# matheusfalcaopinto/triple-hybrid-rag

Measured on AMD Instinct MI355X. Metric: queries/sec (fused top-10), higher is better.
Workload: dtype f16 MFMA shortlist scan (f32 accumulate) + f64 rescoring of the f32 rows

## Files before the change

### triple-hybrid-rag_amd/_native.py

```python
from __future__ import annotations

import ctypes as C
import os
from typing import Optional, Tuple

import torch

from . import _build

THR_FLAG_CERTIFIED = 1
THR_FLAG_OVERFLOW = 2
THR_FLAG_EXACT = 4
THR_DENSE_MAX_K = 256
THR_BM25_MAX_TERMS = 32
THR_BM25_MAX_QUERIES = 1 << 20
THR_GRAPH_MAX_SEEDS = 16
THR_RRF_MAX_PER_CHANNEL = 128
THR_TOPK_MAX = 128
ABI_VERSION = 9

_lib = None


class NativeError(RuntimeError):
# ... 148 lines not shown
def _alloc_out(nq: int, k: int, device):
    tile = torch.empty((2, nq, k), dtype=torch.int64, device=device)
    return (tile[0].view(torch.float64), tile[1],
            torch.empty(nq, dtype=torch.int32, device=device),
            torch.empty(nq, dtype=torch.int32, device=device))


def _coll(doc_coll, query_coll, n: int, nq: int):
    if query_coll is None:
        return None, None
    if doc_coll is None:
        raise NativeError("query_coll without doc_coll")
    if doc_coll.shape != (n,) or query_coll.shape != (nq,):
        raise NativeError("doc_coll / query_coll have the wrong length")
    return _dev(doc_coll, torch.int32, "doc_coll", 1), _dev(query_coll, torch.int32, "query_coll", 1)


def dense_topk(docs, dnorm, inv_norm, queries, k: int, kprime: int, id_base: int = 0,
               workspace: Optional[torch.Tensor] = None, doc_coll=None, query_coll=None):
    pd = _dev(docs, torch.float32, "docs", 2)
    n, d = docs.shape
    pq = _dev(queries, torch.float32, "queries", 2)
    nq = queries.shape[0]
    if queries.shape[1] != d:
        raise NativeError(f"queries dim {queries.shape[1]} != docs dim {d}")
    pn = _dev(dnorm, torch.float64, "dnorm", 1)
    pi = _dev(inv_norm, torch.float32, "inv_norm", 1)
    if dnorm.shape[0] != n or inv_norm.shape[0] != n:
        raise NativeError("dnorm / inv_norm length != n_docs")
    need = dense_workspace_bytes(n, d, nq, kprime)
    if workspace is None or workspace.numel() * workspace.element_size() < need:
        workspace = torch.empty(need, dtype=torch.uint8, device=docs.device)
    pw = _dev(workspace, workspace.dtype, "workspace")
    S, I, cnt, flg = _alloc_out(nq, k, docs.device)
    pdc, pqc = _coll(doc_coll, query_coll, n, nq)
    _check(load().thr_dense_topk(pd, pn, pi, n, d, id_base, pq, nq, k, kprime, pdc, pqc, S.data_ptr(),
                                 I.data_ptr(), cnt.data_ptr(), flg.data_ptr(), pw,
                                 workspace.numel() * workspace.element_size(), _stream()),
           "thr_dense_topk")
    return S, I, cnt, flg


def dense_topk_exact(docs, dnorm, queries, k: int, id_base: int = 0, doc_coll=None, query_coll=None):
    pd = _dev(docs, torch.float32, "docs", 2)
    n, d = docs.shape
    pq = _dev(queries, torch.float32, "queries", 2)
    nq = queries.shape[0]
    if queries.shape[1] != d:
        raise NativeError(f"queries dim {queries.shape[1]} != docs dim {d}")
    pn = _dev(dnorm, torch.float64, "dnorm", 1)
    if dnorm.shape[0] != n:
        raise NativeError("dnorm length != n_docs")
    need = int(load().thr_dense_exact_workspace_bytes(n, nq))
    ws = torch.empty(need, dtype=torch.uint8, device=docs.device)
    S, I, cnt, flg = _alloc_out(nq, k, docs.device)
    pdc, pqc = _coll(doc_coll, query_coll, n, nq)
    _check(load().thr_dense_topk_exact(pd, pn, n, d, id_base, pq, nq, k, pdc, pqc, S.data_ptr(),
                                       I.data_ptr(), cnt.data_ptr(), flg.data_ptr(),
                                       ws.data_ptr(), need, _stream()), "thr_dense_topk_exact")
    return S, I, cnt, flg


def dense_scan_probe(docs, inv_norm, queries, workspace: torch.Tensor) -> None:
    pd = _dev(docs, torch.float32, "docs", 2)
    n, d = docs.shape
    pq = _dev(queries, torch.float32, "queries", 2)
    if queries.shape[1] != d or inv_norm.shape[0] != n:
        raise NativeError("probe: shape mismatch")
    pi = _dev(inv_norm, torch.float32, "inv_norm", 1)
    pw = _dev(workspace, workspace.dtype, "workspace")
    _check(load().thr_dense_scan_probe(pd, pi, n, d, pq, queries.shape[0], pw,
                                       workspace.numel() * workspace.element_size(), _stream()),
           "thr_dense_scan_probe")


def dense_f16_query_tile(dim: int, packed: bool, n_queries: int) -> int:
    return int(load().thr_dense_f16_query_tile(dim, 1 if packed else 0, n_queries))


def dense_f16_max_queries(dim: int, packed: bool) -> int:
    return int(load().thr_dense_f16_max_queries(dim, 1 if packed else 0))


def dense_rescue_workspace_bytes(n_queries: int, k: int) -> int:
    return int(load().thr_dense_rescue_workspace_bytes(n_queries, k))


def dense_rescue(docs, dnorm, queries, S, I, cnt, flg, id_base: int = 0,
                 workspace: Optional[torch.Tensor] = None, doc_coll=None, query_coll=None) -> torch.Tensor:
    pd = _dev(docs, torch.float32, "docs", 2)
    pn = _dev(dnorm, torch.float64, "dnorm", 1)
    pq = _dev(queries, torch.float32, "queries", 2)
    n, d = docs.shape
    nq, k = I.shape
    need = int(load().thr_dense_rescue_workspace_bytes(nq, k))
    if workspace is None or workspace.numel() * workspace.element_size() < need:
        workspace = torch.empty(need, dtype=torch.uint8, device=docs.device)
    n_rescued = torch.zeros(1, dtype=torch.int32, device=docs.device)
    pdc, pqc = _coll(doc_coll, query_coll, n, nq)
    _check(load().thr_dense_rescue(pd, pn, n, d, id_base, pq, nq, k, pdc, pqc, S.data_ptr(), I.data_ptr(),
                                   cnt.data_ptr(), flg.data_ptr(), n_rescued.data_ptr(),
                                   workspace.data_ptr(),
                                   workspace.numel() * workspace.element_size(), _stream()),
           "thr_dense_rescue")
    return n_rescued


def dense_quantize_f16(docs: torch.Tensor, keep_copy: bool = True):
    p = _dev(docs, torch.float32, "docs", 2)
    n, d = docs.shape
    d16 = None
    if keep_copy:
        nbytes = int(load().thr_dense_f16_copy_bytes(n, d))
        d16 = torch.empty((nbytes // (2 * d), d), dtype=torch.float16, device=docs.device)
    err = torch.zeros(1, dtype=torch.float32, device=docs.device)
    _check(load().thr_dense_quantize_f16(p, n, d, d16.data_ptr() if keep_copy else None,
                                         err.data_ptr(), _stream()), "thr_dense_quantize_f16")
    return d16, float(err.item())


def dense_f16_layout(dim: int) -> str:
    return f"fragment-major/mfma{32 if os.environ.get('THR_DENSE_MFMA') == '32' else 16}/dim{dim}"


def dense_f16_workspace_bytes(n_docs: int, dim: int, n_queries: int, kprime: int) -> int:
    return int(load().thr_dense_f16_workspace_bytes(n_docs, dim, n_queries, kprime))


def dense_topk_f16(docs, docs16, doc_rel_err: float, dnorm, inv_norm, queries, k: int,
                   kprime: int, id_base: int = 0, workspace: Optional[torch.Tensor] = None,
                   doc_coll=None, query_coll=None):
    pd = _dev(docs, torch.float32, "docs", 2)
    ph = _dev(docs16, torch.float16, "docs16", 2) if docs16 is not None else None
    n, d = docs.shape
    if docs16 is not None and tuple(docs16.shape) != ((n + 31) // 32 * 32, d):
        raise NativeError("docs16 is not the fragment-major copy of docs (thr_dense_quantize_f16)")
    pq = _dev(queries, torch.float32, "queries", 2)
    nq = queries.shape[0]
    if queries.shape[1] != d:
        raise NativeError(f"queries dim {queries.shape[1]} != docs dim {d}")
    pn = _dev(dnorm, torch.float64, "dnorm", 1)
    pi = _dev(inv_norm, torch.float32, "inv_norm", 1)
    if dnorm.shape[0] != n or inv_norm.shape[0] != n:
        raise NativeError("dnorm / inv_norm length != n_docs")
    need = dense_f16_workspace_bytes(n, d, nq, kprime)
    if workspace is None or workspace.numel() * workspace.element_size() < need:
        workspace = torch.empty(need, dtype=torch.uint8, device=docs.device)
    pw = _dev(workspace, workspace.dtype, "workspace")
    S, I, cnt, flg = _alloc_out(nq, k, docs.device)
    pdc, pqc = _coll(doc_coll, query_coll, n, nq)
    _check(load().thr_dense_topk_f16(pd, ph, float(doc_rel_err), pn, pi, n, d, id_base, pq, nq, k,
                                     kprime, pdc, pqc, S.data_ptr(), I.data_ptr(), cnt.data_ptr(),
                                     flg.data_ptr(), pw,
                                     workspace.numel() * workspace.element_size(), _stream()),
           "thr_dense_topk_f16")
    return S, I, cnt, flg


def dense_shortlist_f16(docs, docs16, doc_rel_err: float, inv_norm, queries, kprime: int, m: int,
                        workspace: torch.Tensor, doc_coll=None, query_coll=None) -> torch.Tensor:
    pd = _dev(docs, torch.float32, "docs", 2)
    ph = _dev(docs16, torch.float16, "docs16", 2) if docs16 is not None else None
    n, d = docs.shape
    pq = _dev(queries, torch.float32, "queries", 2)
    nq = queries.shape[0]
    if queries.shape[1] != d or inv_norm.shape[0] != n:
        raise NativeError("shortlist: shape mismatch")
    pi = _dev(inv_norm, torch.float32, "inv_norm", 1)
    need = dense_f16_workspace_bytes(n, d, nq, kprime)
    if workspace.numel() * workspace.element_size() < need:
        raise NativeError("shortlist: workspace smaller than thr_dense_f16_workspace_bytes")
    pw = _dev(workspace, workspace.dtype, "workspace")
    pdc, pqc = _coll(doc_coll, query_coll, n, nq)
    lb = torch.empty((nq, m), dtype=torch.float32, device=docs.device)
    _check(load().thr_dense_shortlist_f16(pd, ph, float(doc_rel_err), pi, n, d, pq, nq, kprime, pdc, pqc,
                                          m, lb.data_ptr(), pw,
                                          workspace.numel() * workspace.element_size(), _stream()),
           "thr_dense_shortlist_f16")
    return lb


# ... 465 lines not shown
```

### triple-hybrid-rag_amd/csrc/dense.hip

```cpp
#include <stdlib.h>

#include "thr_common.hpp"

namespace thr {

constexpr int CHUNK = 256;
constexpr int MODE_ALL = 0, MODE_FILTER = 1;
constexpr int CAND_CAP = 16384;
constexpr int SAMPLE_MAX = 1 << 20;
constexpr int WBUF = 256;
constexpr int ROW_BITS = 27;
constexpr uint32_t ROW_MASK = (1u << ROW_BITS) - 1;
constexpr int ROW_BITS_F16 = 25;

struct Cand {
    float score;
    uint32_t doc;
};

}
struct ScanSlot {
    int qtile, slice, nslices;
};
__device__ __forceinline__ ScanSlot scan_slot(int n_qtiles) {
// ... 623 lines not shown
                [&](int u) { return fkey(load_cand(u).score); }, my_n, kprime, hist, bc);
            floor32 = fkey_inv(tkey);
            for (int u = 0; u < my_n; ++u) {
                const Cand e = load_cand(u);
                if (fkey(e.score) > tkey) {
                    const int p = atomicAdd(&n_sel, 1);
                    s_id[p] = e.doc;
                }
            }
            __syncthreads();
            for (int u = 0; u < my_n; ++u) {
                const Cand e = load_cand(u);
                if (fkey(e.score) == tkey) {
                    const int p = atomicAdd(&n_sel, 1);
                    if (p < kprime) s_id[p] = e.doc;
                }
            }
            __syncthreads();
            if (threadIdx.x == 0 && n_sel > kprime) n_sel = kprime;
        } else {
            for (int u = 0; u < my_n; ++u) {
                const Cand e = load_cand(u);
                if (e.score > -INFINITY) {
                    const int p = atomicAdd(&n_sel, 1);
                    s_id[p] = e.doc;
                }
            }
        }
    }
    __syncthreads();
    const int ns = n_sel;
    for (int i = threadIdx.x; i < ns; i += SEL_THREADS) sel_rows[(int64_t)q * CAPB + i] = s_id[i];
    if (threadIdx.x == 0) {
        sel_meta[4 * q + 0] = ns;
        sel_meta[4 * q + 1] = (int32_t)__float_as_uint(floor32);
        sel_meta[4 * q + 2] = overflow ? 1 : 0;
        sel_meta[4 * q + 3] = (int32_t)__float_as_uint(gF);
    }
}

constexpr int RR_WAVES = 2, RR_THREADS = 64 * RR_WAVES, RR_ROWS = 64;
static size_t rescore_lds_bytes(int dim) {
    return sizeof(double) * dim + sizeof(float4) * RR_WAVES * RR_ROWS * RS_STRIDE;
}
template <int U>
__device__ __forceinline__ double rescore_pass(const f32x4* (&rp)[8], f32x4* stage, const double* q64,
                                               int nchunk, int lane, int lrow, int lch) {
    constexpr int D = U >= 2 ? 16 / U : 8;
    f32x4 nxt[D][U];
#pragma unroll
    for (int dd = 0; dd < D; ++dd)
#pragma unroll
        for (int u = 0; u < U; ++u) nxt[dd][u] = rp[u][8 * dd];
    double dot = 0.0;
#pragma unroll 1
    for (int ck0 = 0; ck0 < nchunk; ck0 += D) {
#pragma unroll
        for (int dd = 0; dd < D; ++dd) {
            const int ck = ck0 + dd;
#pragma unroll
            for (int u = 0; u < U; ++u) stage[(lrow + 8 * u) * RS_STRIDE + lch] = nxt[dd][u];
            const int cn = ck + D < nchunk ? ck + D : nchunk - 1;
#pragma unroll
            for (int u = 0; u < U; ++u) nxt[dd][u] = rp[u][8 * cn];
            __builtin_amdgcn_fence(__ATOMIC_ACQ_REL, "wavefront");
            __builtin_amdgcn_wave_barrier();
            const f32x4* src = stage + lane * RS_STRIDE;
            const double* qv = q64 + 32 * ck;
#pragma unroll
            for (int ch = 0; ch < 8; ++ch) {
                const f32x4 x = src[ch];
                dot = __fma_rn((double)x.x, qv[4 * ch + 0], dot);
                dot = __fma_rn((double)x.y, qv[4 * ch + 1], dot);
                dot = __fma_rn((double)x.z, qv[4 * ch + 2], dot);
                dot = __fma_rn((double)x.w, qv[4 * ch + 3], dot);
            }
            __builtin_amdgcn_fence(__ATOMIC_ACQ_REL, "wavefront");
            __builtin_amdgcn_wave_barrier();
        }
    }
    return dot;
}

template <int NB>
__global__ __launch_bounds__(RR_THREADS, 3) void rescore_rank(
    const float* __restrict__ docs, const double* __restrict__ dnorm, int dim, int64_t id_base,
    const float* __restrict__ queries, int k, double eps32, double doc_relerr,
    const float* __restrict__ qerr, const int32_t* __restrict__ sel_rows,
    const int32_t* __restrict__ sel_meta, double* __restrict__ out_scores,
    int64_t* __restrict__ out_ids, int32_t* __restrict__ out_counts, uint32_t* __restrict__ out_flags) {
    const int q = blockIdx.x;
    const int ns = sel_meta[4 * q + 0];
    if (NB == THR_DENSE_MAX_K ? ns > THR_DENSE_MAX_K : ns <= THR_DENSE_MAX_K) return;
    const float floor32 = __uint_as_float((uint32_t)sel_meta[4 * q + 1]);
    const bool overflow = sel_meta[4 * q + 2] != 0;
    extern __shared__ float4 lds_sel[];
    __shared__ double s_s[NB], o_s[NB];
    __shared__ int64_t s_id[NB], o_id[NB];
    __shared__ double s_qn;
    __shared__ int n_valid;
    const int lane = threadIdx.x & 63, wave = threadIdx.x >> 6;
    const double eq = qerr ? (double)qerr[q] : 0.0;
    const double eps = eps32 + doc_relerr * (1.0 + eq) + eq;
    double* q64 = reinterpret_cast<double*>(lds_sel);
    for (int i = threadIdx.x; i < dim; i += RR_THREADS) q64[i] = (double)queries[(int64_t)q * dim + i];
    for (int i = threadIdx.x; i < NB; i += RR_THREADS) {
        s_s[i] = o_s[i] = -INFINITY;
        s_id[i] = i < ns ? (int64_t)sel_rows[(int64_t)q * SEL_BIG_BAND + i] : INT64_MAX;
        o_id[i] = INT64_MAX;
    }
    if (threadIdx.x == 0) n_valid = 0;
    __syncthreads();

    f32x4* stage = reinterpret_cast<f32x4*>(lds_sel + dim / 2) + wave * (RR_ROWS * RS_STRIDE);
    const f32x4* docs4 = reinterpret_cast<const f32x4*>(docs);
    const int lrow = lane >> 3, lch = lane & 7;
    const int cpr = dim / 4, nchunk = dim / 32;
    const f32x4* q4 = reinterpret_cast<const f32x4*>(queries + (int64_t)q * dim);
    const double dn_first = (int)threadIdx.x < ns ? dnorm[s_id[threadIdx.x]] : 0.0;
    for (int b0 = 0; b0 <= ns; b0 += RR_WAVES * RR_ROWS) {
        const int rem = ns - b0 - wave;
        if (rem < 0) continue;
        const f32x4* rp[8];
#pragma unroll
        for (int u = 0; u < 8; ++u) {
            int j = b0 + wave + RR_WAVES * (lrow + 8 * u);
            j = j < ns ? j : ns;
            rp[u] = (j < ns ? docs4 + s_id[j] * cpr : q4) + lch;
        }
        const int jm = b0 + wave + RR_WAVES * lane;
        const int groups = rem / RR_WAVES / 8 + 1;
        double dot;
        if (groups <= 1) dot = rescore_pass<1>(rp, stage, q64, nchunk, lane, lrow, lch);
        else if (groups <= 2) dot = rescore_pass<2>(rp, stage, q64, nchunk, lane, lrow, lch);
        else if (groups <= 4) dot = rescore_pass<4>(rp, stage, q64, nchunk, lane, lrow, lch);
        else dot = rescore_pass<8>(rp, stage, q64, nchunk, lane, lrow, lch);
        if (jm < ns) s_s[jm] = dot;
        else if (jm == ns) s_qn = __dsqrt_rn(dot);
    }
    __syncthreads();
    for (int p = threadIdx.x; p < ns; p += RR_THREADS) {
        const int64_t row = s_id[p];
        const double qn = s_qn, dn = p == (int)threadIdx.x ? dn_first : dnorm[row], dot = s_s[p];
        double sim = -INFINITY;
        if (dn > 0.0) sim = qn > 0.0 ? __ddiv_rn(dot, __dmul_rn(qn, dn)) : 0.0;
        s_s[p] = sim;
        s_id[p] = sim == -INFINITY ? INT64_MAX : row + id_base;
    }
    __syncthreads();
    for (int p = threadIdx.x; p < ns; p += RR_THREADS) {
        const double ms = s_s[p];
        const int64_t mi = s_id[p];
        if (mi == INT64_MAX) continue;
        int rank = 0;
        for (int i = 0; i < ns; ++i) rank += better(s_s[i], s_id[i], ms, mi) ? 1 : 0;
        o_s[rank] = ms;
        o_id[rank] = mi;
    }
    __syncthreads();

    int mine_valid = 0;
    for (int i = threadIdx.x; i < k; i += RR_THREADS) {
        const bool ok = o_s[i] > -INFINITY;
        mine_valid += ok ? 1 : 0;
        out_scores[(int64_t)q * k + i] = ok ? o_s[i] : -INFINITY;
        out_ids[(int64_t)q * k + i] = ok ? o_id[i] : -1;
    }
    if (mine_valid) atomicAdd(&n_valid, mine_valid);
    __syncthreads();
    if (threadIdx.x == 0) {
        const int valid = n_valid;
        uint32_t flag = overflow ? THR_FLAG_OVERFLOW : 0u;
        bool cert;
        if (overflow) {
            cert = false;
        } else if (floor32 == -INFINITY) {
            cert = true;
        } else {
            const float gF = __uint_as_float((uint32_t)sel_meta[4 * q + 3]);
            const bool own = valid >= k && s_qn > 0.0 && (o_s[k - 1] - (double)floor32 / s_qn) > eps;
            const bool all = gF > -INFINITY && s_qn > 0.0 &&
                             ((double)gF / s_qn - (double)floor32 / s_qn) > eps;
            cert = own || all;
        }
        out_flags[q] = flag | (cert ? THR_FLAG_CERTIFIED : 0u);
        out_counts[q] = valid;
    }
}

constexpr int EX_THREADS = 256;
constexpr int EX_CAP = 1024;
constexpr int EX_SLABS = 64;

__global__ __launch_bounds__(EX_THREADS) void exact_slab_topk(
    const float* __restrict__ docs, const double* __restrict__ dnorm, int64_t n_docs, int dim,
    const float* __restrict__ queries, int n_queries, int k, double* __restrict__ slab_s,
    int64_t* __restrict__ slab_id, const uint32_t* __restrict__ skip_certified,
    const int32_t* __restrict__ doc_coll, const int32_t* __restrict__ query_coll) {
    extern __shared__ float lds_qv[];
    __shared__ double b_s[EX_CAP];
    __shared__ int64_t b_id[EX_CAP];
    __shared__ int b_cnt;
    __shared__ double t_s;
    __shared__ int64_t t_id;
    __shared__ double s_qn;
    __shared__ unsigned long long s_todo;
    const int slab = blockIdx.x;
    {
        const int q = blockIdx.y + (int)threadIdx.x * (int)gridDim.y;
        const bool todo = threadIdx.x < 64 && q < n_queries &&
                          !(skip_certified && (skip_certified[q] & THR_FLAG_CERTIFIED));
        const unsigned long long m = __ballot(todo);
        if (threadIdx.x == 0) s_todo = m;
        __syncthreads();
    }
    for (unsigned long long todo = s_todo; todo; todo &= todo - 1) {
        const int q = blockIdx.y + (__ffsll((long long)todo) - 1) * (int)gridDim.y;
        __syncthreads();
        for (int i = threadIdx.x; i < dim; i += EX_THREADS) lds_qv[i] = queries[(int64_t)q * dim + i];
        __syncthreads();
        if (threadIdx.x == 0) s_qn = __dsqrt_rn(seq_dot_f64(lds_qv, lds_qv, dim));
        BlockTopK<EX_CAP, EX_THREADS> tk;
        tk.init(b_s, b_id, &b_cnt, &t_s, &t_id, k);
        const double qn = s_qn;
        const int qc = query_coll ? query_coll[q] : -1;
        const int64_t per = (n_docs + EX_SLABS - 1) / EX_SLABS;
        const int64_t lo = slab * per, hi = (lo + per < n_docs) ? lo + per : n_docs;
        for (int64_t base = lo; base < hi; base += EX_THREADS) {
            int64_t row = base + threadIdx.x;
            bool ok = row < hi;
            double sim = -INFINITY;
            if (ok) {
                double dn = dnorm[row];
                if (qc != -1 && doc_coll[row] != qc) dn = 0.0;
                if (dn > 0.0) {
                    double dot = seq_dot_f64(docs + row * dim, lds_qv, dim);
                    sim = qn > 0.0 ? __ddiv_rn(dot, __dmul_rn(qn, dn)) : 0.0;
                }
            }
            tk.push(ok && sim > -INFINITY, sim, row);
        }
        int n = tk.finish();
        for (int i = threadIdx.x; i < k; i += EX_THREADS) {
            int64_t o = ((int64_t)q * EX_SLABS + slab) * k + i;
            slab_s[o] = i < n ? b_s[i] : -INFINITY;
            slab_id[o] = i < n ? b_id[i] : INT64_MAX;
        }
    }
}
// ... 457 lines not shown
                          int n_queries, int k, int kprime, double* out_scores, int64_t* out_ids,
                          int32_t* out_counts, uint32_t* out_flags, char* ws, hipStream_t st,
                          const int32_t* doc_coll, const int32_t* query_coll, int phase = PIPE_ALL,
                          const float* gfloor = nullptr, float* top_lb = nullptr, int top_m = 0,
                          const float* lb_all = nullptr, int n_shards = 0) {
    float* tau = (float*)(ws + p.off_tau);
    const bool h = p.kind == KIND_F16;
    float* qerr = h ? (float*)(ws + p.off_qerr) : nullptr;
    int* cnt = (int*)(ws + p.off_cnt);
    int* tcnt = (int*)(ws + p.off_tcnt);
    Cand* cand = (Cand*)(ws + p.off_cand);
    Cand* tlist = (Cand*)(ws + p.off_tlist);
    float* sample = (float*)(ws + p.off_sample);
    _Float16* qfrag = (_Float16*)(ws + p.off_qfrag);
    int nseg = 0;
    auto scan = [&](bool all, int64_t units, int64_t stride, float* smp, int64_t ld) -> int {
        if (p.qreg)
            return all ? launch_scan_f16q<MODE_ALL>(dim, docs16, qfrag, p.ntiles, units, stride,
                                                    nullptr, nullptr, nullptr, smp, ld, st, nullptr,
                                                    nullptr, nullptr, n_queries)
                       : launch_scan_f16q<MODE_FILTER>(dim, docs16, qfrag, p.ntiles, units, stride,
                                                       tau, cnt, cand, nullptr, 0, st, &nseg, doc_coll,
                                                       query_coll, n_queries);
        if (h)
            return all ? launch_scan_f16<MODE_ALL>(dim, p.nq, docs, inv_norm, n_docs, queries,
                                                   n_queries, p.ntiles, units, stride, nullptr,
                                                   nullptr, nullptr, 0, smp, ld, st)
                       : launch_scan_f16<MODE_FILTER>(dim, p.nq, docs, inv_norm, n_docs, queries,
                                                      n_queries, p.ntiles, units, stride, tau, tcnt,
                                                      tlist, p.tile_cap, nullptr, 0, st, doc_coll, query_coll);
        return all ? launch_scan_mfma<MODE_ALL>(dim, docs, inv_norm, n_docs, queries, n_queries,
                                               p.ntiles, units, stride, nullptr, nullptr, nullptr,
                                               0, smp, ld, st)
                   : launch_scan_mfma<MODE_FILTER>(dim, docs, inv_norm, n_docs, queries, n_queries,
                                                  p.ntiles, units, stride, tau, tcnt, tlist,
                                                  p.tile_cap, nullptr, 0, st, doc_coll, query_coll);
    };
    int rc;
    const double u = 5.9604644775390625e-08;
    const double eps32 = h ? ((double)dim + 16.0) * u : scan_eps(dim);
    int32_t* sel_rows = (int32_t*)(ws + p.off_selrows);
    int32_t* sel_meta = (int32_t*)(ws + p.off_selmeta);
    if (phase == PIPE_FINISH) {
        if (p.qreg && (rc = launch_scan_f16q<MODE_FILTER, true>(dim, docs16, qfrag, p.ntiles, p.groups, 1,
                                                                 nullptr, nullptr, nullptr, nullptr, 0, st,
                                                                 &nseg)))
            return rc;
    } else {
    hipError_t e = hipMemsetAsync(cnt, 0, p.off_cand - p.off_cnt, st);
    if (e != hipSuccess) return (int)e;
    if (p.qreg && (rc = launch_pack_queries(dim, queries, n_queries, p.qpad, qfrag, qerr, st))) return rc;
    float* qerr_k2 = p.qreg ? nullptr : qerr;
    if (p.sampled) {
        if ((rc = scan(true, p.sample_groups, p.sample_stride, sample, p.sample_docs))) return rc;
        hipLaunchKernelGGL(kth_select, dim3(p.qpad), dim3(256), 0, st, sample, p.sample_docs,
                           (int)p.sample_docs, p.ksample, queries, n_queries, dim, tau, qerr_k2,
                           doc_coll, query_coll, p.unit, p.sample_stride, n_docs);
    } else {
        hipLaunchKernelGGL(kth_select, dim3(p.qpad), dim3(256), 0, st, (const float*)nullptr,
                           (int64_t)0, 0, p.ksample, queries, n_queries, dim, tau, qerr_k2,
                           doc_coll, query_coll, p.unit, (int64_t)1, n_docs);
    }
    if ((rc = launch_status())) return rc;
    if ((rc = scan(false, p.groups, 1, nullptr, 0))) return rc;
    if (!p.qreg) {
        hipLaunchKernelGGL(bucket_candidates, dim3(BUCKET_BLOCKS, p.ntiles), dim3(256), 0, st, tcnt,
                           tlist, p.tile_cap, p.qtile, p.row_bits, cnt, cand);
        if ((rc = launch_status())) return rc;
    }
    }
    if (phase == PIPE_SHORTLIST) {
        hipLaunchKernelGGL(select_band<true>, dim3(n_queries), dim3(SEL_THREADS), band_lds_bytes(dim), st,
                           dim, queries, tau, cnt, cand, tcnt, p.tile_cap, p.qtile, k, kprime, eps32,
                           doc_relerr, qerr, nseg, nseg ? CAND_CAP / nseg : 0, doc_coll, query_coll,
                           sel_rows, sel_meta, (const float*)nullptr, (const float*)nullptr, 0, 0, top_lb,
                           top_m);
        return launch_status();
    }
    hipLaunchKernelGGL(select_band<false>, dim3(n_queries), dim3(SEL_THREADS), band_lds_bytes(dim), st,
                       dim, queries, tau, cnt, cand, tcnt, p.tile_cap, p.qtile, k, kprime, eps32,
                       doc_relerr, qerr, nseg, nseg ? CAND_CAP / nseg : 0, doc_coll, query_coll,
                       sel_rows, sel_meta, gfloor, lb_all, n_shards, top_m, (float*)nullptr, 0);
    if ((rc = launch_status())) return rc;
    hipLaunchKernelGGL(rescore_rank<THR_DENSE_MAX_K>, dim3(n_queries), dim3(RR_THREADS),
                       rescore_lds_bytes(dim), st, docs, dnorm, dim, id_base, queries, k, eps32,
                       doc_relerr, qerr, sel_rows, sel_meta, out_scores, out_ids, out_counts, out_flags);
    if ((rc = launch_status())) return rc;
    hipLaunchKernelGGL(rescore_rank<SEL_BIG_BAND>, dim3(n_queries), dim3(RR_THREADS),
                       rescore_lds_bytes(dim), st, docs, dnorm, dim, id_base, queries, k, eps32,
                       doc_relerr, qerr, sel_rows, sel_meta, out_scores, out_ids, out_counts, out_flags);
    return launch_status();
}

static int dense_args_ok(const void* docs, const void* dnorm, const void* inv_norm,
                         const void* queries, const void* a, const void* b, const void* c,
                         const void* d, const void* ws, int64_t n_docs, int n_queries, int k,
                         int kprime) {
    THR_RETURN_IF(!docs || !dnorm || !inv_norm || !queries || !a || !b || !c || !d || !ws,
                  THR_ERR_INVALID);
    THR_RETURN_IF(n_docs <= 0 || n_queries <= 0 || k <= 0 || kprime < k ||
                      kprime > THR_DENSE_MAX_K,
                  THR_ERR_INVALID);
    return THR_OK;
}

extern "C" int thr_dense_topk(const float* docs, const double* dnorm, const float* inv_norm,
                              int64_t n_docs, int dim, int64_t id_base, const float* queries,
                              int n_queries, int k, int kprime, const int32_t* doc_coll,
                              const int32_t* query_coll, double* out_scores,
                              int64_t* out_ids, int32_t* out_counts, uint32_t* out_flags,
                              void* workspace, size_t workspace_bytes, thr_stream_t stream) {
    clear_status();
    int rc = dense_args_ok(docs, dnorm, inv_norm, queries, out_scores, out_ids, out_counts,
                           out_flags, workspace, n_docs, n_queries, k, kprime);
    if (rc) return rc;
    THR_RETURN_IF((query_coll != nullptr) != (doc_coll != nullptr), THR_ERR_INVALID);
    THR_RETURN_IF(dim <= 0 || dim % CHUNK != 0 || dim / CHUNK > 4, THR_ERR_UNSUPPORTED);
    THR_RETURN_IF(n_docs >= (int64_t)1 << ROW_BITS, THR_ERR_UNSUPPORTED);
    const DensePlan p = make_plan(n_docs, n_queries, kprime);
    THR_RETURN_IF(workspace_bytes < p.total, THR_ERR_WORKSPACE);
    return dense_pipeline(p, docs, nullptr, 0.0, dnorm, inv_norm, n_docs, dim, id_base, queries,
                          n_queries, k, kprime, out_scores, out_ids, out_counts, out_flags,
                          (char*)workspace, (hipStream_t)stream, doc_coll, query_coll);
}

extern "C" size_t thr_dense_f16_workspace_bytes(int64_t n_docs, int dim, int n_queries,
                                                int kprime) {
    if (n_docs <= 0 || n_queries <= 0) return 0;
    const size_t a = make_plan(n_docs, n_queries, kprime, KIND_F16, dim, false).total;
    const size_t b = make_plan(n_docs, n_queries, kprime, KIND_F16, dim, true).total;
    return a > b ? a : b;
}

extern "C" int thr_dense_f16_max_queries(int dim, int packed) {
    if (dim != 512 && dim != 768 && dim != 1024) return 0;
    return packed ? qreg_max_queries(dim) : INT32_MAX;
}

extern "C" int thr_dense_f16_query_tile(int dim, int packed, int n_queries) {
    if (dim != 512 && dim != 768 && dim != 1024) return 0;
    (void)n_queries;
    return packed ? qreg_qw(dim) * qreg_waves(dim) : 32 * f16_pick_nq(dim);
}

extern "C" size_t thr_dense_f16_copy_bytes(int64_t n_docs, int dim) {
    if (n_docs <= 0 || dim <= 0) return 0;
    return sizeof(_Float16) * (size_t)((n_docs + 31) / 32 * 32) * (size_t)dim;
}

extern "C" int thr_dense_quantize_f16(const float* docs, int64_t n_docs, int dim, uint16_t* docs16,
                                      float* max_rel_err, thr_stream_t stream) {
    clear_status();
    THR_RETURN_IF(!docs || !max_rel_err || n_docs <= 0 || dim <= 0, THR_ERR_INVALID);
    THR_RETURN_IF(dim % 64 != 0, THR_ERR_UNSUPPORTED);
    hipStream_t st = (hipStream_t)stream;
    hipError_t e = hipMemsetAsync(max_rel_err, 0, sizeof(float), st);
    if (e != hipSuccess) return (int)e;
    if (docs16) {
        THR_RETURN_IF(dim % 16 != 0, THR_ERR_UNSUPPORTED);
        const int64_t n_pad = (n_docs + 31) / 32 * 32;
        hipLaunchKernelGGL(quantize_f16_norm, dim3((unsigned)((n_pad + 3) / 4)), dim3(256), 0, st,
                           docs, n_docs, dim, qreg_shape(dim), reinterpret_cast<_Float16*>(docs16),
                           reinterpret_cast<unsigned int*>(max_rel_err));
        return launch_status();
    }
    hipLaunchKernelGGL(measure_f16_error, dim3((unsigned)((n_docs + 3) / 4)), dim3(256), 0, st, docs,
                       n_docs, dim, reinterpret_cast<unsigned int*>(max_rel_err));
    return launch_status();
}

extern "C" int thr_dense_topk_f16(const float* docs, const uint16_t* docs16, double doc_rel_err,
// ... 254 lines not shown
```

### triple-hybrid-rag_amd/csrc/rrf.hip

```cpp
#include "thr_common.hpp"

namespace thr {

constexpr int RRF_THREADS = 128;
constexpr int RRF_MAXC = THR_RRF_MAX_PER_CHANNEL;
constexpr int RRF_SLOTS = 512;

__device__ __forceinline__ int last_rank(const int64_t* l, int n, int64_t id) {
    int r = 0;
    for (int j = 0; j < n; ++j)
        if (l[j] == id) r = j + 1;
    return r;
}
__device__ __forceinline__ bool seen_before(const int64_t* l, int i, int64_t id) {
    for (int j = 0; j < i; ++j)
        if (l[j] == id) return true;
    return false;
}

constexpr int RRF_RAG2 = 0, RRF_STANDALONE = 1, RRF_TWO = 2;
__device__ __forceinline__ int occurrences(const int64_t* l, int n, int64_t id) {
    int c = 0;
    for (int j = 0; j < n; ++j) c += l[j] == id ? 1 : 0;
    return c;
}

template <int MODE>
__global__ __launch_bounds__(RRF_THREADS) void rrf_fuse_kernel(
    const int64_t* __restrict__ lex, int n_lex, const int64_t* __restrict__ sem, int n_sem,
    const int64_t* __restrict__ gra, int n_gra, double w_lex, double w_sem, double w_gra, int rrf_k,
    int top_k, int64_t* __restrict__ out_ids, double* __restrict__ out_scores,
    int32_t* __restrict__ out_ranks, int32_t* __restrict__ out_counts) {
    static_assert(RRF_THREADS == RRF_MAXC && RRF_THREADS == 2 * WAVE, "one thread per position");
    __shared__ int64_t L[3][RRF_MAXC];
    __shared__ int len[3];
    __shared__ int wave_new[3][2];
    __shared__ double s_s[RRF_SLOTS];
    __shared__ int64_t c_id[RRF_SLOTS];
    __shared__ int c_rank[RRF_SLOTS][3];
    __shared__ int order[RRF_SLOTS];

    const int q = blockIdx.x, t = threadIdx.x, lane = t & 63, wave = t >> 6;
    const int64_t* src[3] = {lex, sem, gra};
    const int width[3] = {lex ? n_lex : 0, sem ? n_sem : 0, gra ? n_gra : 0};
    if (t < 3) len[t] = width[t];
    __syncthreads();
    for (int ch = 0; ch < 3; ++ch) {
        const int64_t id = t < width[ch] ? src[ch][(int64_t)q * width[ch] + t] : -1;
        L[ch][t] = id;
        if (t < width[ch] && id < 0) atomicMin(&len[ch], t);
    }
    __syncthreads();

    bool nw[3];
    int within[3];
    for (int ch = 0; ch < 3; ++ch) {
        nw[ch] = false;
        if (t < len[ch]) {
            const int64_t id = L[ch][t];
            nw[ch] = !seen_before(L[ch], t, id);
            for (int e = 0; e < ch && nw[ch]; ++e)
                if (last_rank(L[e], len[e], id)) nw[ch] = false;
        }
        const uint64_t m = __ballot(nw[ch]);
        within[ch] = __popcll(m & ((1ull << lane) - 1ull));
        if (lane == 0) wave_new[ch][wave] = __popcll(m);
    }
    __syncthreads();
    int base = 0, n = 0;
    for (int ch = 0; ch < 3; ++ch) {
        const int here = base + (wave ? wave_new[ch][0] : 0) + within[ch];
        base += wave_new[ch][0] + wave_new[ch][1];
        if (!nw[ch]) continue;
        const int64_t id = L[ch][t];
        const int lr = last_rank(L[0], len[0], id);
        const int sr = last_rank(L[1], len[1], id);
        const int gr = last_rank(L[2], len[2], id);
        double score = 0.0;
        if (MODE == RRF_RAG2) {
            if (lr) score = __dadd_rn(score, __ddiv_rn(w_lex, (double)(rrf_k + lr)));
            if (sr) score = __dadd_rn(score, __ddiv_rn(w_sem, (double)(rrf_k + sr)));
            if (gr) score = __dadd_rn(score, __ddiv_rn(w_gra, (double)(rrf_k + gr)));
        } else {
            const double w[3] = {w_lex, w_sem, w_gra};
            const int rk[3] = {lr, sr, gr};
#pragma unroll
            for (int c = 0; c < 3; ++c)
                if (rk[c]) {
                    const double v = __dmul_rn(w[c], __ddiv_rn(1.0, (double)(rrf_k + rk[c])));
                    const int reps = (MODE == RRF_TWO && c == 0) ? 1 : occurrences(L[c], len[c], id);
                    for (int r = 0; r < reps; ++r) score = __dadd_rn(score, v);
                }
        }
        c_id[here] = id;
        c_rank[here][0] = lr;
        c_rank[here][1] = sr;
        c_rank[here][2] = gr;
        s_s[here] = score;
    }
    n = base;
    __syncthreads();
    for (int p = t; p < n; p += RRF_THREADS) {
        const double ms = s_s[p];
        int rank = 0;
        for (int j = 0; j < n; ++j) {
            const double o = s_s[j];
            rank += (o > ms || (o == ms && j < p)) ? 1 : 0;
        }
        order[rank] = p;
    }
    __syncthreads();
    for (int i = t; i < top_k; i += RRF_THREADS) {
        const bool ok = i < n;
        const int p = ok ? order[i] : 0;
        out_ids[(int64_t)q * top_k + i] = ok ? c_id[p] : -1;
        out_scores[(int64_t)q * top_k + i] = ok ? s_s[p] : -INFINITY;
        if (out_ranks)
            for (int c = 0; c < 3; ++c)
                out_ranks[((int64_t)q * top_k + i) * 3 + c] = ok ? c_rank[p][c] : 0;
    }
    if (t == 0) out_counts[q] = n < top_k ? n : top_k;
}

__global__ __launch_bounds__(RRF_THREADS) void rerank_order_kernel(
    const float* __restrict__ scores, int n_lists, int64_t list_stride,
    const int64_t* __restrict__ ids, const int32_t* __restrict__ counts, int n, int top_k,
    int64_t* __restrict__ out_ids, double* __restrict__ out_scores, int32_t* __restrict__ out_counts) {
    __shared__ double s_s[RRF_SLOTS];
    __shared__ int order[RRF_SLOTS];
    const int q = blockIdx.x, t = threadIdx.x;
    int cnt = counts ? counts[q] : n;
    cnt = cnt < n ? cnt : n;
    for (int p = t; p < cnt; p += RRF_THREADS) {
        float best = -INFINITY;
        for (int l = 0; l < n_lists; ++l) best = fmaxf(best, scores[(int64_t)l * list_stride + (int64_t)q * n + p]);
        s_s[p] = best > -INFINITY ? (double)best : 0.0;
    }
    __syncthreads();
    for (int p = t; p < cnt; p += RRF_THREADS) {
        const double ms = s_s[p];
        int rank = 0;
        for (int j = 0; j < cnt; ++j) {
            const double o = s_s[j];
            rank += (o > ms || (o == ms && j < p)) ? 1 : 0;
        }
        order[rank] = p;
    }
    __syncthreads();
    for (int i = t; i < top_k; i += RRF_THREADS) {
        const bool ok = i < cnt;
        const int p = ok ? order[i] : 0;
        out_ids[(int64_t)q * top_k + i] = ok ? ids[(int64_t)q * n + p] : -1;
        out_scores[(int64_t)q * top_k + i] = ok ? s_s[p] : -INFINITY;
    }
    if (t == 0) out_counts[q] = cnt < top_k ? cnt : top_k;
}

__global__ __launch_bounds__(RRF_THREADS) void fuse_post_kernel(
    const int64_t* __restrict__ ids, const double* __restrict__ scores,
    const int32_t* __restrict__ ranks, const int32_t* __restrict__ counts, int n,
    const double* __restrict__ lex_s, int n_lex, const double* __restrict__ sem_s, int n_sem,
    const double* __restrict__ gra_s, int n_gra, double safety_threshold, int denoise,
    double quantile, int normalize, int top_k, int64_t* __restrict__ out_ids,
    double* __restrict__ out_scores, int32_t* __restrict__ out_counts) {
    __shared__ double s_s[2][RRF_SLOTS];
    __shared__ int64_t s_id[2][RRF_SLOTS];
    __shared__ int wave_cnt[2];
    __shared__ double red[2][2];
    const int q = blockIdx.x, t = threadIdx.x, lane = t & 63, wave = t >> 6;
    int cnt = counts ? counts[q] : n;
    cnt = cnt < n ? cnt : n;
    auto compact = [&](int from, int m, auto keep) -> int {
        int base = 0;
        for (int b0 = 0; b0 < m; b0 += RRF_THREADS) {
            const int i = b0 + t;
            const bool k = i < m && keep(i);
            const uint64_t bal = __ballot(k);
            if (lane == 0) wave_cnt[wave] = __popcll(bal);
            __syncthreads();
            const int at = base + (wave ? wave_cnt[0] : 0) + __popcll(bal & ((1ull << lane) - 1ull));
            if (k) {
                s_s[from ^ 1][at] = s_s[from][i];
                s_id[from ^ 1][at] = s_id[from][i];
            }
            base += wave_cnt[0] + wave_cnt[1];
            __syncthreads();
        }
        return base;
    };
    const double* chs[3] = {lex_s, sem_s, gra_s};
    const int chw[3] = {n_lex, n_sem, n_gra};
    for (int i = t; i < cnt; i += RRF_THREADS) {
        s_s[0][i] = scores[(int64_t)q * n + i];
        s_id[0][i] = ids[(int64_t)q * n + i];
    }
    __syncthreads();
    int m = cnt, cur = 0;
    if (safety_threshold > 0.0 && ranks) {
        m = compact(0, cnt, [&](int i) {
            double best = 0.0;
            for (int c = 0; c < 3; ++c) {
                const int r = ranks[((int64_t)q * n + i) * 3 + c];
                if (r > 0 && chs[c]) {
                    const double v = chs[c][(int64_t)q * chw[c] + r - 1];
                    best = v > best ? v : best;
                }
            }
            return best >= safety_threshold;
        });
        cur = 1;
    }
    if (denoise && m >= 3) {
        const double v = __dmul_rn((double)(m - 1), quantile);
        int prev = (int)floor(v);
        prev = prev < 0 ? 0 : prev > m - 1 ? m - 1 : prev;
        const int next = prev + 1 > m - 1 ? m - 1 : prev + 1;
        const double g = __dsub_rn(v, (double)prev);
        const double a = s_s[cur][m - 1 - prev], bb = s_s[cur][m - 1 - next];
        const double diff = __dsub_rn(bb, a);
        const double cut = g >= 0.5 ? __dsub_rn(bb, __dmul_rn(diff, __dsub_rn(1.0, g)))
                                    : __dadd_rn(a, __dmul_rn(diff, g));
        __syncthreads();
        const int from = cur;
        m = compact(from, m, [&](int i) { return s_s[from][i] >= cut; });
        cur ^= 1;
    }
    if (top_k > 0 && m > top_k) m = top_k;
    double lo = 0.0, hi = 0.0;
    if (normalize && m > 0) {
        double mn = INFINITY, mx = -INFINITY;
// ... 115 lines not shown
```

Baseline: 737,100.

## Hash-dedupe RRF candidates, merge rescore kernels, pool zero counters

RRF fusion replaces quadratic linear scans for duplicate detection, last rank and occurrence counting with a shared-memory open-addressing hash table. The rank sort is register-blocked over several positions per thread. The two templated rescore_rank launches collapse into one kernel that uses 32-bit row ids and reuses the stage LDS for its outputs. A pooled zero tensor replaces a per-call torch.zeros allocation. Together these cut launches, allocation and O(n^2) work, at the cost of atomics in the hash insert and a pooled counter slice whose reuse must stay correct.

```diff
diff --git a/triple-hybrid-rag_amd/_native.py b/triple-hybrid-rag_amd/_native.py
--- a/triple-hybrid-rag_amd/_native.py
+++ b/triple-hybrid-rag_amd/_native.py
@@ -254,6 +254,17 @@
     return int(load().thr_dense_f16_max_queries(dim, 1 if packed else 0))
 
 
+_ZERO_POOL: dict = {}
+
+
+def _zero_i32(device) -> torch.Tensor:
+    pool = _ZERO_POOL.get(str(device))
+    if pool is None or pool[1] >= pool[0].numel():
+        pool = _ZERO_POOL[str(device)] = [torch.zeros(4096, dtype=torch.int32, device=device), 0]
+    pool[1] += 1
+    return pool[0][pool[1] - 1:pool[1]]
+
+
 def dense_rescue_workspace_bytes(n_queries: int, k: int) -> int:
     return int(load().thr_dense_rescue_workspace_bytes(n_queries, k))
 
@@ -268,7 +279,7 @@
     need = int(load().thr_dense_rescue_workspace_bytes(nq, k))
     if workspace is None or workspace.numel() * workspace.element_size() < need:
         workspace = torch.empty(need, dtype=torch.uint8, device=docs.device)
-    n_rescued = torch.zeros(1, dtype=torch.int32, device=docs.device)
+    n_rescued = _zero_i32(docs.device)
     pdc, pqc = _coll(doc_coll, query_coll, n, nq)
     _check(load().thr_dense_rescue(pd, pn, n, d, id_base, pq, nq, k, pdc, pqc, S.data_ptr(), I.data_ptr(),
                                    cnt.data_ptr(), flg.data_ptr(), n_rescued.data_ptr(),
diff --git a/triple-hybrid-rag_amd/csrc/dense.hip b/triple-hybrid-rag_amd/csrc/dense.hip
--- a/triple-hybrid-rag_amd/csrc/dense.hip
+++ b/triple-hybrid-rag_amd/csrc/dense.hip
@@ -729,7 +729,6 @@
     return dot;
 }
 
-template <int NB>
 __global__ __launch_bounds__(RR_THREADS, 3) void rescore_rank(
     const float* __restrict__ docs, const double* __restrict__ dnorm, int dim, int64_t id_base,
     const float* __restrict__ queries, int k, double eps32, double doc_relerr,
@@ -737,13 +736,15 @@
     const int32_t* __restrict__ sel_meta, double* __restrict__ out_scores,
     int64_t* __restrict__ out_ids, int32_t* __restrict__ out_counts, uint32_t* __restrict__ out_flags) {
     const int q = blockIdx.x;
-    const int ns = sel_meta[4 * q + 0];
-    if (NB == THR_DENSE_MAX_K ? ns > THR_DENSE_MAX_K : ns <= THR_DENSE_MAX_K) return;
+    constexpr int NB = SEL_BIG_BAND, NOUT = THR_DENSE_MAX_K;
+    const int ns = sel_meta[4 * q + 0] < NB ? sel_meta[4 * q + 0] : NB;
     const float floor32 = __uint_as_float((uint32_t)sel_meta[4 * q + 1]);
     const bool overflow = sel_meta[4 * q + 2] != 0;
     extern __shared__ float4 lds_sel[];
-    __shared__ double s_s[NB], o_s[NB];
-    __shared__ int64_t s_id[NB], o_id[NB];
+    __shared__ double s_s[NB];
+    __shared__ int32_t s_id[NB];
+    static_assert(sizeof(float4) * RR_WAVES * RR_ROWS * RS_STRIDE >= NOUT * (sizeof(double) + sizeof(int32_t)),
+                  "the ranked output fits the stage tiles");
     __shared__ double s_qn;
     __shared__ int n_valid;
     const int lane = threadIdx.x & 63, wave = threadIdx.x >> 6;
@@ -751,10 +752,9 @@
     const double eps = eps32 + doc_relerr * (1.0 + eq) + eq;
     double* q64 = reinterpret_cast<double*>(lds_sel);
     for (int i = threadIdx.x; i < dim; i += RR_THREADS) q64[i] = (double)queries[(int64_t)q * dim + i];
-    for (int i = threadIdx.x; i < NB; i += RR_THREADS) {
-        s_s[i] = o_s[i] = -INFINITY;
-        s_id[i] = i < ns ? (int64_t)sel_rows[(int64_t)q * SEL_BIG_BAND + i] : INT64_MAX;
-        o_id[i] = INT64_MAX;
+    for (int i = threadIdx.x; i < ns; i += RR_THREADS) {
+        s_s[i] = -INFINITY;
+        s_id[i] = sel_rows[(int64_t)q * SEL_BIG_BAND + i];
     }
     if (threadIdx.x == 0) n_valid = 0;
     __syncthreads();
@@ -773,7 +773,7 @@
         for (int u = 0; u < 8; ++u) {
             int j = b0 + wave + RR_WAVES * (lrow + 8 * u);
             j = j < ns ? j : ns;
-            rp[u] = (j < ns ? docs4 + s_id[j] * cpr : q4) + lch;
+            rp[u] = (j < ns ? docs4 + (int64_t)s_id[j] * cpr : q4) + lch;
         }
         const int jm = b0 + wave + RR_WAVES * lane;
         const int groups = rem / RR_WAVES / 8 + 1;
@@ -786,23 +786,31 @@
         else if (jm == ns) s_qn = __dsqrt_rn(dot);
     }
     __syncthreads();
+    double* o_s = reinterpret_cast<double*>(lds_sel + dim / 2);
+    int32_t* o_id = reinterpret_cast<int32_t*>(o_s + NOUT);
+    for (int i = threadIdx.x; i < NOUT; i += RR_THREADS) {
+        o_s[i] = -INFINITY;
+        o_id[i] = INT32_MAX;
+    }
     for (int p = threadIdx.x; p < ns; p += RR_THREADS) {
-        const int64_t row = s_id[p];
+        const int32_t row = s_id[p];
         const double qn = s_qn, dn = p == (int)threadIdx.x ? dn_first : dnorm[row], dot = s_s[p];
         double sim = -INFINITY;
         if (dn > 0.0) sim = qn > 0.0 ? __ddiv_rn(dot, __dmul_rn(qn, dn)) : 0.0;
         s_s[p] = sim;
-        s_id[p] = sim == -INFINITY ? INT64_MAX : row + id_base;
+        s_id[p] = sim == -INFINITY ? INT32_MAX : row;
     }
     __syncthreads();
     for (int p = threadIdx.x; p < ns; p += RR_THREADS) {
         const double ms = s_s[p];
-        const int64_t mi = s_id[p];
-        if (mi == INT64_MAX) continue;
+        const int32_t mi = s_id[p];
+        if (mi == INT32_MAX) continue;
         int rank = 0;
         for (int i = 0; i < ns; ++i) rank += better(s_s[i], s_id[i], ms, mi) ? 1 : 0;
-        o_s[rank] = ms;
-        o_id[rank] = mi;
+        if (rank < NOUT) {
+            o_s[rank] = ms;
+            o_id[rank] = mi;
+        }
     }
     __syncthreads();
 
@@ -811,7 +819,7 @@
         const bool ok = o_s[i] > -INFINITY;
         mine_valid += ok ? 1 : 0;
         out_scores[(int64_t)q * k + i] = ok ? o_s[i] : -INFINITY;
-        out_ids[(int64_t)q * k + i] = ok ? o_id[i] : -1;
+        out_ids[(int64_t)q * k + i] = ok ? (int64_t)o_id[i] + id_base : -1;
     }
     if (mine_valid) atomicAdd(&n_valid, mine_valid);
     __syncthreads();
@@ -1435,11 +1443,7 @@
                        doc_relerr, qerr, nseg, nseg ? CAND_CAP / nseg : 0, doc_coll, query_coll,
                        sel_rows, sel_meta, gfloor, lb_all, n_shards, top_m, (float*)nullptr, 0);
     if ((rc = launch_status())) return rc;
-    hipLaunchKernelGGL(rescore_rank<THR_DENSE_MAX_K>, dim3(n_queries), dim3(RR_THREADS),
-                       rescore_lds_bytes(dim), st, docs, dnorm, dim, id_base, queries, k, eps32,
-                       doc_relerr, qerr, sel_rows, sel_meta, out_scores, out_ids, out_counts, out_flags);
-    if ((rc = launch_status())) return rc;
-    hipLaunchKernelGGL(rescore_rank<SEL_BIG_BAND>, dim3(n_queries), dim3(RR_THREADS),
+    hipLaunchKernelGGL(rescore_rank, dim3(n_queries), dim3(RR_THREADS),
                        rescore_lds_bytes(dim), st, docs, dnorm, dim, id_base, queries, k, eps32,
                        doc_relerr, qerr, sel_rows, sel_meta, out_scores, out_ids, out_counts, out_flags);
     return launch_status();
diff --git a/triple-hybrid-rag_amd/csrc/rrf.hip b/triple-hybrid-rag_amd/csrc/rrf.hip
--- a/triple-hybrid-rag_amd/csrc/rrf.hip
+++ b/triple-hybrid-rag_amd/csrc/rrf.hip
@@ -6,24 +6,44 @@
 constexpr int RRF_MAXC = THR_RRF_MAX_PER_CHANNEL;
 constexpr int RRF_SLOTS = 512;
 
-__device__ __forceinline__ int last_rank(const int64_t* l, int n, int64_t id) {
-    int r = 0;
-    for (int j = 0; j < n; ++j)
-        if (l[j] == id) r = j + 1;
-    return r;
-}
-__device__ __forceinline__ bool seen_before(const int64_t* l, int i, int64_t id) {
-    for (int j = 0; j < i; ++j)
-        if (l[j] == id) return true;
-    return false;
+constexpr uint64_t RRF_EMPTY = ~0ull;
+
+__device__ __forceinline__ int rrf_slot(uint64_t* hkey, int64_t id) {
+    uint32_t h = ((uint32_t)id ^ (uint32_t)((uint64_t)id >> 32)) * 2654435761u >> (32 - __builtin_ctz(RRF_SLOTS));
+    for (;;) {
+        const uint64_t old = atomicCAS((unsigned long long*)&hkey[h], (unsigned long long)RRF_EMPTY,
+                                       (unsigned long long)id);
+        if (old == RRF_EMPTY || old == (uint64_t)id) return (int)h;
+        h = (h + 1) & (RRF_SLOTS - 1);
+    }
+}
+
+template <int NI>
+__device__ __forceinline__ void rrf_rank_sort(const double* s_s, int n, int* order, int t) {
+    double ms[NI];
+    int rank[NI];
+#pragma unroll
+    for (int i = 0; i < NI; ++i) {
+        const int p = t + i * RRF_THREADS;
+        ms[i] = p < n ? s_s[p] : 0.0;
+        rank[i] = 0;
+    }
+    for (int j = 0; j < n; j += 2) {
+        const double o0 = s_s[j], o1 = s_s[j + 1];
+        const bool two = j + 1 < n;
+#pragma unroll
+        for (int i = 0; i < NI; ++i) {
+            const int p = t + i * RRF_THREADS;
+            rank[i] += (o0 > ms[i] || (o0 == ms[i] && j < p)) ? 1 : 0;
+            rank[i] += (two && (o1 > ms[i] || (o1 == ms[i] && j + 1 < p))) ? 1 : 0;
+        }
+    }
+#pragma unroll
+    for (int i = 0; i < NI; ++i)
+        if (t + i * RRF_THREADS < n) order[rank[i]] = t + i * RRF_THREADS;
 }
 
 constexpr int RRF_RAG2 = 0, RRF_STANDALONE = 1, RRF_TWO = 2;
-__device__ __forceinline__ int occurrences(const int64_t* l, int n, int64_t id) {
-    int c = 0;
-    for (int j = 0; j < n; ++j) c += l[j] == id ? 1 : 0;
-    return c;
-}
 
 template <int MODE>
 __global__ __launch_bounds__(RRF_THREADS) void rrf_fuse_kernel(
@@ -32,36 +52,50 @@
     int top_k, int64_t* __restrict__ out_ids, double* __restrict__ out_scores,
     int32_t* __restrict__ out_ranks, int32_t* __restrict__ out_counts) {
     static_assert(RRF_THREADS == RRF_MAXC && RRF_THREADS == 2 * WAVE, "one thread per position");
-    __shared__ int64_t L[3][RRF_MAXC];
+    static_assert(RRF_SLOTS > 3 * RRF_MAXC, "the hash set keeps a free slot");
+    constexpr int NCAND = 3 * RRF_MAXC;
+    __shared__ uint64_t hkey[RRF_SLOTS];
+    __shared__ int hfirst[RRF_SLOTS];
+    __shared__ int hrank[RRF_SLOTS][3];
+    __shared__ int hocc[MODE == RRF_RAG2 ? 1 : RRF_SLOTS][3];
     __shared__ int len[3];
     __shared__ int wave_new[3][2];
-    __shared__ double s_s[RRF_SLOTS];
-    __shared__ int64_t c_id[RRF_SLOTS];
-    __shared__ int c_rank[RRF_SLOTS][3];
-    __shared__ int order[RRF_SLOTS];
+    __shared__ __align__(16) double s_s[NCAND + 2];
+    __shared__ int c_slot[NCAND];
+    __shared__ int order[NCAND];
 
     const int q = blockIdx.x, t = threadIdx.x, lane = t & 63, wave = t >> 6;
     const int64_t* src[3] = {lex, sem, gra};
     const int width[3] = {lex ? n_lex : 0, sem ? n_sem : 0, gra ? n_gra : 0};
     if (t < 3) len[t] = width[t];
-    __syncthreads();
+    for (int i = t; i < RRF_SLOTS; i += RRF_THREADS) {
+        hkey[i] = RRF_EMPTY;
+        hfirst[i] = NCAND;
+        hrank[i][0] = hrank[i][1] = hrank[i][2] = 0;
+        if (MODE != RRF_RAG2) hocc[i][0] = hocc[i][1] = hocc[i][2] = 0;
+    }
+    __syncthreads();
+    int64_t id[3];
     for (int ch = 0; ch < 3; ++ch) {
-        const int64_t id = t < width[ch] ? src[ch][(int64_t)q * width[ch] + t] : -1;
-        L[ch][t] = id;
-        if (t < width[ch] && id < 0) atomicMin(&len[ch], t);
+        id[ch] = t < width[ch] ? src[ch][(int64_t)q * width[ch] + t] : -1;
+        if (t < width[ch] && id[ch] < 0) atomicMin(&len[ch], t);
+    }
+    __syncthreads();
+    int slot[3];
+    for (int ch = 0; ch < 3; ++ch) {
+        slot[ch] = -1;
+        if (t >= len[ch]) continue;
+        const int s = slot[ch] = rrf_slot(hkey, id[ch]);
+        atomicMin(&hfirst[s], ch * RRF_MAXC + t);
+        atomicMax(&hrank[s][ch], t + 1);
+        if (MODE != RRF_RAG2) atomicAdd(&hocc[s][ch], 1);
     }
     __syncthreads();
 
     bool nw[3];
     int within[3];
     for (int ch = 0; ch < 3; ++ch) {
-        nw[ch] = false;
-        if (t < len[ch]) {
-            const int64_t id = L[ch][t];
-            nw[ch] = !seen_before(L[ch], t, id);
-            for (int e = 0; e < ch && nw[ch]; ++e)
-                if (last_rank(L[e], len[e], id)) nw[ch] = false;
-        }
+        nw[ch] = slot[ch] >= 0 && hfirst[slot[ch]] == ch * RRF_MAXC + t;
         const uint64_t m = __ballot(nw[ch]);
         within[ch] = __popcll(m & ((1ull << lane) - 1ull));
         if (lane == 0) wave_new[ch][wave] = __popcll(m);
@@ -72,10 +106,8 @@
         const int here = base + (wave ? wave_new[ch][0] : 0) + within[ch];
         base += wave_new[ch][0] + wave_new[ch][1];
         if (!nw[ch]) continue;
-        const int64_t id = L[ch][t];
-        const int lr = last_rank(L[0], len[0], id);
-        const int sr = last_rank(L[1], len[1], id);
-        const int gr = last_rank(L[2], len[2], id);
+        const int s = slot[ch];
+        const int lr = hrank[s][0], sr = hrank[s][1], gr = hrank[s][2];
         double score = 0.0;
         if (MODE == RRF_RAG2) {
             if (lr) score = __dadd_rn(score, __ddiv_rn(w_lex, (double)(rrf_k + lr)));
@@ -88,36 +120,28 @@
             for (int c = 0; c < 3; ++c)
                 if (rk[c]) {
                     const double v = __dmul_rn(w[c], __ddiv_rn(1.0, (double)(rrf_k + rk[c])));
-                    const int reps = (MODE == RRF_TWO && c == 0) ? 1 : occurrences(L[c], len[c], id);
+                    const int reps = (MODE == RRF_TWO && c == 0) ? 1 : hocc[s][c];
                     for (int r = 0; r < reps; ++r) score = __dadd_rn(score, v);
                 }
         }
-        c_id[here] = id;
-        c_rank[here][0] = lr;
-        c_rank[here][1] = sr;
-        c_rank[here][2] = gr;
+        c_slot[here] = s;
         s_s[here] = score;
     }
     n = base;
     __syncthreads();
-    for (int p = t; p < n; p += RRF_THREADS) {
-        const double ms = s_s[p];
-        int rank = 0;
-        for (int j = 0; j < n; ++j) {
-            const double o = s_s[j];
-            rank += (o > ms || (o == ms && j < p)) ? 1 : 0;
-        }
-        order[rank] = p;
-    }
+    if (n <= RRF_THREADS) rrf_rank_sort<1>(s_s, n, order, t);
+    else if (n <= 2 * RRF_THREADS) rrf_rank_sort<2>(s_s, n, order, t);
+    else rrf_rank_sort<3>(s_s, n, order, t);
     __syncthreads();
     for (int i = t; i < top_k; i += RRF_THREADS) {
         const bool ok = i < n;
         const int p = ok ? order[i] : 0;
-        out_ids[(int64_t)q * top_k + i] = ok ? c_id[p] : -1;
+        const int s = ok ? c_slot[p] : 0;
+        out_ids[(int64_t)q * top_k + i] = ok ? (int64_t)hkey[s] : -1;
         out_scores[(int64_t)q * top_k + i] = ok ? s_s[p] : -INFINITY;
         if (out_ranks)
             for (int c = 0; c < 3; ++c)
-                out_ranks[((int64_t)q * top_k + i) * 3 + c] = ok ? c_rank[p][c] : 0;
+                out_ranks[((int64_t)q * top_k + i) * 3 + c] = ok ? hrank[s][c] : 0;
     }
     if (t == 0) out_counts[q] = n < top_k ? n : top_k;
 }
@@ -126,7 +150,7 @@
     const float* __restrict__ scores, int n_lists, int64_t list_stride,
     const int64_t* __restrict__ ids, const int32_t* __restrict__ counts, int n, int top_k,
     int64_t* __restrict__ out_ids, double* __restrict__ out_scores, int32_t* __restrict__ out_counts) {
-    __shared__ double s_s[RRF_SLOTS];
+    __shared__ __align__(16) double s_s[RRF_SLOTS + 2];
     __shared__ int order[RRF_SLOTS];
     const int q = blockIdx.x, t = threadIdx.x;
     int cnt = counts ? counts[q] : n;
@@ -137,15 +161,8 @@
         s_s[p] = best > -INFINITY ? (double)best : 0.0;
     }
     __syncthreads();
-    for (int p = t; p < cnt; p += RRF_THREADS) {
-        const double ms = s_s[p];
-        int rank = 0;
-        for (int j = 0; j < cnt; ++j) {
-            const double o = s_s[j];
-            rank += (o > ms || (o == ms && j < p)) ? 1 : 0;
-        }
-        order[rank] = p;
-    }
+    if (cnt <= RRF_THREADS) rrf_rank_sort<1>(s_s, cnt, order, t);
+    else rrf_rank_sort<RRF_SLOTS / RRF_THREADS>(s_s, cnt, order, t);
     __syncthreads();
     for (int i = t; i < top_k; i += RRF_THREADS) {
         const bool ok = i < cnt;
```

Result: no change. 741,700, median of 6 (+0.6%).
